# RalphAS/PeriodicSchurDecompositions.jl

Measured on AMD Instinct MI355X. Metric: PSD sweeps/sec (pschur! n=1024 p=64 Float64, Hessenberg+Q+iteration, operands in HBM), higher is better.
Workload: dtype f64

## Files before the change

### periodicschurdecompositions.jl_amd/csrc/psd_engine.cpp

```cpp
#include <atomic>
#include "psd_hess.h"
#include "psd_bhess.h"
#include "psd_hess2.h"
#include "psd_formq2.h"
#include "psd_real_qr.h"
#include "psd_apply2.h"
#include "psd_zhess.h"
#include "psd_zhess2.h"
#include "psd_zqz.h"
#include "psd_zord.h"
#include "psd_rord.h"
#include "psd_rgz.h"
#include "psd_zgz.h"
#include "psd_zgord.h"
#include "psd_grord.h"
#include "psd_rhessx.h"
#include "psd_check.h"
#include "psd_krylov.h"
#include "psd_evec.h"
#include "psd_gevec.h"
#include "psd_bevec.h"

#include "../../include/psd_mi355x.h"

// ... 193 lines not shown
    int hess_graph_n = 0, hess_graph_p = 0;
    double* h2ring = nullptr;
    int h2ring_n = 0;
    double* zh2ring = nullptr;
    int zh2ring_n = 0;
    std::vector<hipEvent_t> h2ev;
    int hess_async = -1;
    int hess_lookahead = 1;
    int hess_xcd = 1;
#endif
    int shard_rank = 0, shard_world = 1;
    int batch_group = 0;
    int bh_nmax = PSD_BH_NMAX;
    int bev_nmax = PSD_BEV_NMAX;
    void slice(int p, int& lo, int& hi) const {
        const int base = p / shard_world, rem = p % shard_world;
        lo = shard_rank * base + (shard_rank < rem ? shard_rank : rem);
        hi = lo + base + (shard_rank < rem ? 1 : 0);
    }
    int train_stop = 1;
    int train_wdiv = 0;
    int train_long = 256;
    int band_helper = 1;
    int zstream = 3;
    int zcdefer = 0;
    int redge = 0, cedge = 0;
    int rdefer = 1;
    int cdefer = 1;
    int overlap = 3;
    int far_grid = 0;
    bool counted = false;
    bool pipe_ok = false;
#ifndef PSD_HOSTSIM
    hipStream_t stream2 = nullptr;
    hipStream_t stream3 = nullptr;
    hipStream_t stream4 = nullptr;
    int hess_pipe_depth = 3;
    int hess_pipe = 1;
    hipEvent_t evE[2] = {nullptr, nullptr}, evF[2] = {nullptr, nullptr}, evG[2] = {nullptr, nullptr};
    hipEvent_t evC[2] = {nullptr, nullptr};
#endif
    int apply_worklist = 1;
    int apply_wl_grid = 2048;
    int ncu = 0;
    int slices = 1;
    unsigned char* slmem = nullptr;
// ... 778 lines not shown
        PSD_CHECK(hipFuncSetAttribute(reinterpret_cast<const void*>(psd_rq_step),
                                      hipFuncAttributeMaxDynamicSharedMemorySize, (int)lds_step));
        c->step_lds_set = lds_step;
    }
#endif
    const int M = (c->train_m >= 2) ? ((c->train_m > PSD_TRAIN_MAX) ? PSD_TRAIN_MAX : c->train_m) : 1;
    P.cst = nullptr;
    P.tshift = nullptr;
    P.lead = c->st;
    P.tick = 0;
    P.gl = nullptr;
    P.cep = nullptr;
    P.role = P.epoch = P.cdone = nullptr;
    P.nprob = 1;
    P.ticklog = nullptr;
    P.ticklog_n = 0;
    P.bandinfo = nullptr;
    P.ccancel = nullptr;
    P.plan = nullptr;
    const bool scan3 = c->chase3 && p >= PSD_C3_MINP && p <= PSD_C3_MAXP;
    P.c2off = (scan3 || (c->chase2 && p >= PSD_C2_MINP)) ? (int)((size_t)p * psd_win_area(W) * sizeof(double)) : 0;
    P.c3off = scan3 ? (int)step_lds_scratch_end(p, W, 8, true) : 0;
    P.cdefer = 0;
    P.slG = 1;
    P.slmem = nullptr;
    P.slerr = nullptr;
    const int c2waves = scan3 ? PSD_C3_WAVES : (P.c2off ? 2 : 1);
    (void)c2waves;
    struct ExitGuard {
        psd_ctx* c;
        int** ticklog;
        ~ExitGuard() {
#ifndef PSD_HOSTSIM
            if (c->stream2) (void)hipStreamSynchronize(c->stream2);
#endif
            if (*ticklog) {
                psd_rt_free(*ticklog);
                *ticklog = nullptr;
            }
        }
    } exit_guard{c, &P.ticklog};
    const char* ticklog_path = psd_env_diag("PSD_TICKLOG");
    const int ticklog_cap = 1 << 16;
    if (ticklog_path && nprob == 1) {
        if (psd_rt_malloc((void**)&P.ticklog, sizeof(int) * ticklog_cap) == 0) {
            PSD_CHECK(psd_rt_memset(P.ticklog, 0, sizeof(int) * ticklog_cap, c->stream));
// ... 299 lines not shown
#endif
#ifndef PSD_HOSTSIM
    PSD_CHECK(poller.finish(pend));
#endif
    PSD_CHECK(psd_rt_last_error());
#ifndef PSD_HOSTSIM
    if (slG > 1) {
        int serr = 0;
        PSD_CHECK(psd_rt_d2h(&serr, P.slerr, sizeof(int), c->stream));
        PSD_CHECK(psd_rt_sync(c->stream));
        if (serr) {
            *st_out = hst;
            return PSD_INFO_RUNTIME + 0xfffa;
        }
    }
#endif
    if (P.ticklog) {
        std::vector<int> tl((size_t)ticklog_cap);
        PSD_CHECK(psd_rt_d2h(tl.data(), P.ticklog, sizeof(int) * ticklog_cap, c->stream));
        PSD_CHECK(psd_rt_sync(c->stream));
        fprintf(stderr, "psd ticklog: phase cycles (decide, spawn, train shifts, small QR, claims, cursor states, deflate, RQ window):");
        for (int q = 0; q < 8; ++q) fprintf(stderr, " %lld/%d", hgl.dbg[q], hgl.dbgn[q]);
        fprintf(stderr, "\n");
        if (hgl.c3dbg[7] > 0) {
            fprintf(stderr, "psd ticklog: scan chase, cycles per position (loads + scan 1, reflectors + B, scan 2, 2-reflectors + records, barrier, apply 0, apply 1) over %lld positions:", hgl.c3dbg[7]);
            for (int q = 0; q < 7; ++q) fprintf(stderr, " %.0f", (double)hgl.c3dbg[q] / (double)hgl.c3dbg[7]);
            fprintf(stderr, "\n");
        }
        if (FILE* fh = fopen(ticklog_path, "w")) {
            for (long long t = 0; t < launched && t < ticklog_cap; ++t) fprintf(fh, "%lld %d %d\n", t, tl[(size_t)t] >> 12, tl[(size_t)t] & 0xfff);
            fclose(fh);
        }
    }
    *st_out = hst;
    if (stats) {
        stats->nlaunch_step = (int32_t)launched;
        stats->window = W;
        stats->step_kernel_ms_avg = samples ? sample_ms / samples : 0.0;
        stats->step_kernel_samples = samples;
    }
    return 0;
}

void stats_from_state(psd_stats* s, const psd_rstate& st) {
    if (!s) return;
    s->niter = st.niter;
// ... 121 lines not shown
        if (const char* e = psd_env("PSD_H2_PIPE")) c->hess_pipe = atoi(e);
        if (const char* e = psd_env("PSD_H2_DEPTH")) c->hess_pipe_depth = atoi(e);
    }
#endif
#ifndef PSD_HOSTSIM
    if (const char* e = psd_env("PSD_HESS_LOOKAHEAD")) c->hess_lookahead = atoi(e);
    if (const char* e = psd_env("PSD_HESS_ASYNC")) c->hess_async = atoi(e);
#endif
#ifdef PSD_HOSTSIM
    if (const char* e = psd_env("PSD_OVERLAP")) c->overlap = atoi(e);
#endif
    if (const char* e = psd_env("PSD_CDEFER")) c->cdefer = atoi(e);
    if (const char* e = psd_env("PSD_RDEFER")) c->rdefer = atoi(e);
    if (const char* e = psd_env("PSD_ZCDEFER")) c->zcdefer = atoi(e);
    if (const char* e = psd_env("PSD_ZSTREAM")) c->zstream = atoi(e);
    if (const char* e = psd_env("PSD_RDEFER_EDGE")) c->redge = atoi(e);
    if (const char* e = psd_env("PSD_CDEFER_EDGE")) c->cedge = atoi(e);
    if (const char* e = psd_env("PSD_ORD_PIPE")) c->ord_pipe = atoi(e);
    if (const char* e = psd_env("PSD_FORMQ_BLOCKED")) c->formq_blocked = atoi(e);
    if (const char* e = psd_env("PSD_BATCH_GROUP")) c->batch_group = atoi(e) > 0 ? atoi(e) : 0;
    if (const char* e = psd_env_diag("PSD_BH_NMAX")) c->bh_nmax = (atoi(e) >= 1 && atoi(e) <= 2048) ? atoi(e) : PSD_BH_NMAX;
    if (const char* e = psd_env_diag("PSD_BEV_NMAX")) c->bev_nmax = (atoi(e) >= 1 && atoi(e) <= 2048) ? atoi(e) : PSD_BEV_NMAX;
    if (const char* e = psd_env("PSD_BAND_HELPER")) c->band_helper = atoi(e);
    if (const char* e = psd_env_diag("PSD_TRAIN_LONG")) c->train_long = atoi(e);
    if (const char* e = psd_env_diag("PSD_TRAIN_STOP")) c->train_stop = atoi(e);
    if (const char* e = psd_env_diag("PSD_TRAIN_WDIV")) c->train_wdiv = atoi(e) > 0 ? atoi(e) : 0;
    if (const char* e = psd_env("PSD_MB")) c->mblock = atoi(e);
    if (const char* e = psd_env_diag("PSD_TRAIN_MB")) c->train_mb_m = atoi(e);
    if (const char* e = psd_env_diag("PSD_APPLY_WL")) c->apply_worklist = atoi(e);
    if (const char* e = psd_env_diag("PSD_APPLY_WL_GRID")) c->apply_wl_grid = atoi(e) > 0 ? atoi(e) : 2048;
    if (const char* e = psd_env_diag("PSD_APPLY_WL2")) c->apply_wl2 = atoi(e);
    if (const char* e = psd_env("PSD_C2")) c->chase2 = atoi(e);
    if (const char* e = psd_env("PSD_C3")) c->chase3 = atoi(e);
#ifndef PSD_HOSTSIM
#endif
    if (const char* e = psd_env_diag("PSD_APPLY_WL2_GRID")) c->apply_wl2_grid = atoi(e) > 0 ? atoi(e) : 1024;
#ifdef PSD_HOSTSIM
    c->apply_wl_grid = 3;
#endif
    if (const char* e = psd_env("PSD_TRAIN")) c->train_m = c->ztrain_m = c->gtrain_m = atoi(e);
    if (const char* e = psd_env("PSD_TRAIN_Z")) c->ztrain_m = atoi(e);
    if (const char* e = psd_env("PSD_TRAIN_G")) c->gtrain_m = atoi(e);
    c->counted = true;
    c->pipe_ok = g_live_contexts.fetch_add(1) == 0;
    *ctx = c;
    return 0;
// ... 2244 lines not shown
```

### periodicschurdecompositions.jl_amd/csrc/psd_real_qr.h

```cpp
#pragma once
#include "psd_scalar.h"
#include "psd_hqr.h"

enum {
    PSD_PH_DECIDE = 0,
    PSD_PH_RQ = 1,
    PSD_PH_SHIFT = 2,
    PSD_PH_QR = 3,
    PSD_PH_DEFLATE = 4,
    PSD_PH_NEXT = 5,
    PSD_PH_FINAL = 6,
    PSD_PH_DONE = 7,
    PSD_PH_TWAIT = 8,
    PSD_PH_CWAIT = 9,
    PSD_PH_CDONE = 10
};
enum { PSD_TR_R3 = 3, PSD_TR_H2 = 2, PSD_TR_R2 = 4, PSD_TR_G = 5 };

#define PSD_TR_CAP 64
#define PSD_STEP_NT 64
#define PSD_APPLY_NT 128
#define PSD_TRAIN_MAX 64
#define PSD_SLOTS 64
enum { PSD_ROLE_FREE = 0, PSD_ROLE_CLAIMED = 1, PSD_ROLE_LEADER = 2, PSD_ROLE_CURSOR = 3 };
// ... 71 lines not shown
    int exc_dec;
    int mb, slot, parent, lo, train_key;
    int prob;
    int cgap, tgap, cstart, cfirst;
    int cslots[PSD_TRAIN_MAX];
    int train_S, train_ms, train_long, train_wdiv;
    int plan_tick, plan_used;
    int opn_tick;
};

struct psd_rglobal {
    int done, info, abort;
    int nactive;
    int nlog;
    int train_seq;
    int itbudget;
    int pactive[PSD_SLOTS], pbudget[PSD_SLOTS], pinfo[PSD_SLOTS];
    int nsweeps, nrqpass, ndefl1, ndefl2, nwindows, ntrains, ntrainsweeps, maxits, nspawn, nslotmax;
    long long niter;
    long long cyc[6];
    long long dbg[8];
    int dbgn[8];
    long long c3dbg[8];
};

struct psd_rparams {
    double* H;
    double* Z;
    psd_rstate* st;
    psd_apply_desc* desc;
    psd_tr* tr;
    int* cnt;
    double* hdiag;
    double* hsub;
    double* hsup;
    double* Pd;
    double* Pe;
    double* Pf;
    double* hnorms;
    double* wr;
    double* wi;
    int* log;
    psd_rstate* cst;
    double* tshift;
    psd_rstate* lead;
    int tick;
    psd_rglobal* gl;
    int* cep;
    int* role;
    int* epoch;
    int nprob;
    int* cdone;
    int* ticklog;
    int ticklog_n;
    int* bandinfo;
    int* ccancel;
    int* plan;
    int c2off;
    int c3off;
    int slG;
    unsigned char* slmem;
    int* slerr;
    int cdefer;
    int redge, cedge;
};
PSD_HD int psd_cdefer_edge(int Wmax) { return (Wmax + 2 > 16) ? (Wmax + 2) : 16; }
PSD_HD int psd_rdefer_edge(int Wmax) { return (2 * Wmax + 8 > 48) ? (2 * Wmax + 8) : 48; }
#define PSD_PLAN_FIRST 0
#define PSD_PLAN_COUNT (PSD_SLOTS)
#define PSD_PLAN_FREE (2 * PSD_SLOTS)
#define PSD_PLAN_CDONE (3 * PSD_SLOTS)
#define PSD_PLAN_CCANCEL (4 * PSD_SLOTS)
#define PSD_PLAN_TICK (5 * PSD_SLOTS)
#define PSD_PLAN_INTS (5 * PSD_SLOTS + 8)
#define PSD_TSHIFT_STRIDE (4 * PSD_TRAIN_MAX + 8)
#define PSD_TRAIN_LONG_MINW 64
#define PSD_DECIDE_YIELD 128

#define PSD_DBG_T0() const long long _dbg0 = (P.ticklog != nullptr) ? psd_clock() : 0
#define PSD_DBG_ADD(k)                                                        \
    do {                                                                      \
        if (P.ticklog != nullptr && P.gl != nullptr) {                        \
            PSD_ONE {                                                         \
                psd_atomic_add_ll(&P.gl->dbg[k], psd_clock() - _dbg0);        \
                psd_atomic_add(&P.gl->dbgn[k], 1);                            \
            }                                                                 \
        }                                                                     \
    } while (0)
PSD_HD psd_mat<double> psd_fac(const psd_rparams& P, int n, int j) {
    return psd_mat<double>{P.H + (size_t)(j - 1) * n * n, n};
}

PSD_HD int psd_win_area(int Wmax) { return Wmax * ((((Wmax + 1) & 1) == 0) ? (Wmax + 1) : (Wmax + 2)); }
PSD_HD int psd_win_pitch(int W, int Wmax) {
    if (((W + 1) & 1) == 0) return W + 1;
    return (W * (W + 2) <= psd_win_area(Wmax)) ? (W + 2) : (W + 1);
}
struct psd_win {
    double* b;
    int W, ld, bsz, bs, be;
    PSD_HD double& at(int j, int r, int c) const { return b[(j - 1) * bsz + (c - bs) * ld + (r - bs)]; }
};

#define PSD_WIN_BAND 3
#define PSD_WIN_LF 4
struct alignas(8) psd_pair {
    double a, b;
};
#ifdef PSD_HOSTSIM
PSD_D psd_pair psd_pair_load(const double* q) { return *(const psd_pair*)q; }
PSD_D void psd_pair_store(double* q, const psd_pair& x) { *(psd_pair*)q = x; }
// ... 430 lines not shown
        const int a = a0 + t;
        if (a <= i) {
            double d = 1.0, e = 0.0, f = 0.0;
            for (int j = 2; j <= p; ++j) {
                const psd_mat<double> Hj = psd_mat<double>{H + (size_t)(j - 1) * n * n, n};
                if (a + 2 <= i) f = d * Hj(a, a + 2) + e * Hj(a + 1, a + 2) + f * Hj(a + 2, a + 2);
                if (a + 1 <= i) e = d * Hj(a, a + 1) + e * Hj(a + 1, a + 1);
                d *= Hj(a, a);
            }
            P.Pd[sb + a] = d;
            P.Pe[sb + a] = e;
            P.Pf[sb + a] = f;
        }
    }
    if (chunk == 0) {
        PSD_ONE {
            P.bandinfo[s] = P.tick;
            P.bandinfo[PSD_SLOTS + s] = lo;
            P.bandinfo[2 * PSD_SLOTS + s] = i;
        }
    }
}

PSD_D double psd_h1_opnorm(const psd_rparams& P, const psd_rstate& st, double* red, int lo, int hi) {
    const psd_mat<double> H1 = psd_fac(P, st.n, 1);
    const int NT = PSD_NTHREADS;
    PSD_PAR_FOR(t, NT) {
        double best = 0.0;
        for (int c = lo + t; c <= hi; c += NT) {
            double s = 0.0;
            const int rmax = (c + 1 < hi) ? (c + 1) : hi;
            for (int r = lo; r <= rmax; ++r) s += fabs(H1(r, c));
            if (s > best) best = s;
        }
        red[t] = best;
    }
    PSD_SYNC();
    double best = 0.0;
    for (int t = 0; t < NT; ++t)
        if (red[t] > best) best = red[t];
    PSD_SYNC();
    return best;
}

PSD_D bool psd_rq_decide(const psd_rparams& P, psd_rstate& st, double* red, int* redi, double* stage, size_t stage_doubles) {
    const int n = st.n, p = st.p, i = st.i, lo = st.l;
    const int NT = PSD_NTHREADS;
    if (!(st.its < st.maxitleft)) {
        if (st.mb && P.nprob > 1) {
            PSD_ONE { psd_atomic_store(&P.gl->pinfo[st.prob], i); }
            st.phase = PSD_PH_FINAL;
            return false;
        }
        st.info = i;
        st.phase = PSD_PH_DONE;
        if (st.mb) {
            PSD_ONE {
                psd_atomic_store(&P.gl->info, i);
                psd_atomic_store(&P.gl->pinfo[st.prob], i);
                psd_atomic_store(&P.gl->abort, 1);
                psd_atomic_store(&P.gl->done, 1);
            }
        }
        return false;
    }
    const psd_mat<double> H1 = psd_fac(P, n, 1);
    bool have = false;
    if (P.bandinfo != nullptr && st.mb) {
        have = P.bandinfo[st.slot] == P.tick && P.bandinfo[PSD_SLOTS + st.slot] <= lo && i <= P.bandinfo[2 * PSD_SLOTS + st.slot];
    }
    if (!have) {
        const int pj = p - 1;
        int R = (pj > 0) ? (int)(stage_doubles / (3 * (size_t)pj)) - 2 : NT;
        if (R > NT) R = NT;
        if (pj > 0 && R >= 1) {
            for (int a0 = lo; a0 <= i; a0 += R) {
                const int a1 = (a0 + R - 1 < i) ? (a0 + R - 1) : i;
                const int c1 = (a1 + 2 < i) ? (a1 + 2) : i;
                const int nc = c1 - a0 + 1;
                PSD_SYNC();
                PSD_PAR_FOR(t, nc * pj) {
                    const int cc = t % nc, jj = t / nc;
                    const int c = a0 + cc;
                    const psd_mat<double> Hj = psd_fac(P, n, jj + 2);
                    double* q = stage + 3 * (size_t)t;
                    q[0] = Hj(c, c);
                    q[1] = (c - 1 >= lo) ? Hj(c - 1, c) : 0.0;
                    q[2] = (c - 2 >= lo) ? Hj(c - 2, c) : 0.0;
                }
// ... 9 lines not shown
                    }
                    P.Pd[a] = d;
                    P.Pe[a] = e;
                    P.Pf[a] = f;
                }
            }
        } else {
            PSD_PAR_FOR(t, i - lo + 1) {
                const int a = lo + t;
                double d = 1.0, e = 0.0, f = 0.0;
                for (int j = 2; j <= p; ++j) {
                    const psd_mat<double> Hj = psd_fac(P, n, j);
                    if (a + 2 <= i) f = d * Hj(a, a + 2) + e * Hj(a + 1, a + 2) + f * Hj(a + 2, a + 2);
                    if (a + 1 <= i) e = d * Hj(a, a + 1) + e * Hj(a + 1, a + 1);
                    d *= Hj(a, a);
                }
                P.Pd[a] = d;
                P.Pe[a] = e;
                P.Pf[a] = f;
            }
        }
    }
    PSD_SYNC();
    PSD_PAR_FOR(t, i - lo + 1) {
        const int r = lo + t;
        if (i == lo) {
            P.hdiag[i] = H1(i, i) * P.Pd[i];
        } else if (r == i) {
            P.hsub[i] = H1(i, i - 1) * P.Pd[i - 1];
            P.hdiag[i] = H1(i, i - 1) * P.Pe[i - 1] + H1(i, i) * P.Pd[i];
        } else if (r > lo) {
            P.hsub[r] = H1(r, r - 1) * P.Pd[r - 1];
            P.hdiag[r] = H1(r, r - 1) * P.Pe[r - 1] + H1(r, r) * P.Pd[r];
            P.hsup[r] = H1(r, r - 1) * P.Pf[r - 1] + H1(r, r) * P.Pe[r] + H1(r, r + 1) * P.Pd[r + 1];
        } else {
            P.hdiag[r] = H1(r, r) * P.Pd[r];
            P.hsup[r] = H1(r, r) * P.Pe[r] + H1(r, r + 1) * P.Pd[r + 1];
        }
    }
    PSD_SYNC();
    int klast = 0;
    double h1norm = -1.0;
    for (int pass = 0; pass < 2; ++pass) {
        PSD_PAR_FOR(t, NT) {
            int best = 0, need = 0;
            for (int k = i - t; k >= lo + 1; k -= NT) {
                const double hh21 = P.hsub[k], hh22 = P.hdiag[k], hh11 = P.hdiag[k - 1], hh12 = P.hsup[k - 1];
                double tst1 = fabs(hh11) + fabs(hh22);
                if (tst1 == 0) {
                    if (h1norm < 0) {
                        need = 1;
                        continue;
                    }
                    tst1 = h1norm;
                }
                bool found = false;
                if (fabs(hh21) <= st.smlnum) {
                    found = true;
                } else if (fabs(hh21) <= st.ulp * tst1) {
                    const double ab = fmax(fabs(hh21), fabs(hh12));
                    const double ba = fmin(fabs(hh21), fabs(hh12));
                    const double aa = fmax(fabs(hh22), fabs(hh11 - hh22));
                    const double bb = fmin(fabs(hh22), fabs(hh11 - hh22));
                    const double stmp = aa + ab;
                    found = ba * (ab / stmp) <= fmax(st.smlnum, st.ulpx * (bb * (aa / stmp)));
                }
                if (found) {
                    best = k;
                    break;
                }
            }
            redi[t] = best;
            redi[NT + t] = need;
        }
        PSD_SYNC();
        int need = 0;
        klast = 0;
        for (int t = 0; t < NT; ++t) {
            if (redi[t] > klast) klast = redi[t];
            need |= redi[NT + t];
        }
        PSD_SYNC();
        if (!need) break;
        if (P.cdefer && st.opn_tick != P.tick - 1) {
            st.opn_tick = P.tick;
            return true;
        }
        h1norm = psd_h1_opnorm(P, st, red, lo, i);
    }
    const bool found = klast > 0;
    const int l = (i > lo) ? (found ? klast : lo) : i;
    st.l = l;
    st.phase = PSD_PH_SHIFT;
    if (l > 1 && st.wantT) {
        double tst1 = fabs(H1(l - 1, l - 1)) + fabs(H1(l, l));
        if (tst1 == 0) {
            if (P.cdefer && st.opn_tick != P.tick - 1) {
                st.opn_tick = P.tick;
                st.l = lo;
                st.phase = PSD_PH_DECIDE;
                return true;
            }
            tst1 = psd_h1_opnorm(P, st, red, l, i);
        }
        if (fabs(H1(l, l - 1)) > fmax(st.ulp * tst1, st.smlnum)) {
            st.phase = PSD_PH_RQ;
            st.kcur = i;
            st.nrqpass += 1;
            psd_log(P, st, 1, l, i);
        } else {
            PSD_SYNC();
            PSD_ONE { H1(l, l - 1) = 0.0; }
            PSD_SYNC();
        }
    }
    return false;
}


PSD_D void psd_rq_startvec(const double h11, const double h12, const double h21, const double h22, const double h32,
                           const double* sh, double* v) {
    const double rt1r = sh[0], rt1i = sh[1], rt2r = sh[2], rt2i = sh[3];
    const double s = fabs(h11 - rt2r) + fabs(rt2i) + fabs(h21);
    const double h21s = h21 / s;
    const double v1 = h21s * h12 + (h11 - rt1r) * ((h11 - rt2r) / s) - rt1i * (rt2i / s);
    const double v2 = h21s * (h11 + h22 - rt1r - rt2r);
    const double v3 = h21s * h32;
    const double t = fabs(v1) + fabs(v2) + fabs(v3);
    v[0] = v1 / t;
    v[1] = v2 / t;
    v[2] = v3 / t;
}

PSD_D void psd_rq_topband(const psd_rparams& P, int n, int p, int l, int i, double& h11, double& h12, double& h21,
                          double& h22, double& h32) {
    double d0 = 1.0, e0 = 0.0, d1 = 1.0;
    for (int j = 2; j <= p; ++j) {
// ... 4 lines not shown
    }
    const psd_mat<double> H1 = psd_fac(P, n, 1);
    h11 = H1(l, l) * d0;
    h12 = H1(l, l) * e0 + H1(l, l + 1) * d1;
    h21 = H1(l + 1, l) * d0;
    h22 = H1(l + 1, l) * e0 + H1(l + 1, l + 1) * d1;
    h32 = (l + 2 <= i) ? H1(l + 2, l + 1) * d1 : 0.0;
}

PSD_HD size_t psd_rq_train_doubles(int p, int m) {
    const size_t K = 2 * (size_t)m, K1 = K + 1;
    return (size_t)p * K1 * K1 + 2 * K1 * K1 + K * K + 3 * PSD_HQR_MAX + 8;
}
PSD_D void psd_rq_train_shifts(const psd_rparams& P, int n, int p, int i, int m, double* work, int* okf) {
    const int K = 2 * m, K1 = K + 1, t0 = i - K + 1, KK = K1 * K1;
    double* B = work;
    double* R0 = B + (size_t)p * KK;
    double* R1 = R0 + KK;
    double* T = R1 + KK;
    double* wr = T + K * K;
    double* wi = wr + PSD_HQR_MAX;
    double* re = wi + PSD_HQR_MAX;
    PSD_SYNC();
    PSD_PAR_FOR(t, p * KK) {
        const int j = t / KK, q = t - j * KK, r = q / K1, c = q - r * K1;
        B[t] = psd_fac(P, n, j + 1)(t0 - 1 + r, t0 - 1 + c);
    }
    PSD_PAR_FOR(q, KK) { R0[q] = (q / K1 == q % K1) ? 1.0 : 0.0; }
    PSD_SYNC();
    double* cur = R0;
    double* nxt = R1;
    for (int j = 2; j <= p; ++j) {
        const double* Bj = B + (size_t)(j - 1) * KK;
        PSD_PAR_FOR(q, KK) {
            const int r = q / K1, c = q - r * K1;
            double acc = 0.0;
            for (int k = r; k <= c; ++k) acc += cur[r * K1 + k] * Bj[k * K1 + c];
            nxt[q] = acc;
        }
        PSD_SYNC();
        double* sw = cur;
        cur = nxt;
        nxt = sw;
    }
    PSD_PAR_FOR(q, K * K) {
        const int r = q / K, c = q - r * K;
        double acc = 0.0;
        for (int k = r; k <= c + 1; ++k) acc += B[(r + 1) * K1 + k] * cur[k * K1 + (c + 1)];
        T[q] = acc;
    }
    PSD_SYNC();
#ifndef PSD_HOSTSIM
    const long long _hq0 = psd_clock();
    const bool okw = psd_hqr_wave(T, K, K, wr, wi, PSD_TID);
    if (P.ticklog != nullptr && P.gl != nullptr) {
        PSD_ONE {
            psd_atomic_add_ll(&P.gl->dbg[3], psd_clock() - _hq0);
            psd_atomic_add(&P.gl->dbgn[3], 1);
        }
    }
#endif
    PSD_ONE {
#ifndef PSD_HOSTSIM
        bool ok = okw;
#else
        bool ok = psd_hqr(T, K, K, wr, wi);
#endif
        int np = 0, nre = 0;
        for (int q = 0; ok && q < K; ++q) {
            if (!(wr[q] == wr[q]) || !(wi[q] == wi[q])) ok = false;
            if (wi[q] > 0.0) {
                if (np < m) {
// ... 14 lines not shown
            }
            re[b + 1] = x;
        }
        for (int a = 0; ok && a < nre && np < m; a += 2) {
            double* sh = P.tshift + 4 * np;
            sh[0] = re[a]; sh[1] = 0.0; sh[2] = (a + 1 < nre) ? re[a + 1] : re[a]; sh[3] = 0.0;
            ++np;
        }
        *okf = (ok && np == m) ? 1 : 0;
    }
    PSD_SYNC();
}

PSD_HD void psd_cursor_schedule(const psd_rstate& st, int b, int& cstart, int& cfirst) {
    const int nbw = st.W - 4;
    const int spc = (st.tgap == 1) ? (nbw + 4) : (2 * nbw);
    int d = (b * spc - nbw + 1 + nbw - 1) / nbw;
    if (d < 1) d = 1;
    int x = nbw * d - b * spc + nbw;
    if (x > nbw) x = nbw;
    if (x < 1) x = 1;
    cstart = st.train_tick0 + d;
    cfirst = x;
}

PSD_D bool psd_rq_shift(const psd_rparams& P, psd_rstate& st, double* work, int* bc) {
    const int n = st.n, i = st.i, l = st.l;
    bool heavy = false;
    if (st.mb && st.l > st.lo && st.l < i - 1) {
        PSD_DBG_T0();
        psd_mb_spawn(P, st, bc);
        PSD_DBG_ADD(1);
    }
    if (l >= i - 1) {
        st.phase = PSD_PH_DEFLATE;
        return false;
    }
    if (!st.wantT) {
        st.i1 = l;
        st.i2 = i;
    }
    psd_log(P, st, 0, l, i);
    st.nsweeps += 1;
    const double dat1 = 0.75, dat2 = -0.4375;
    const double* hdiag = P.hdiag;
    const double* hsub = P.hsub;
// ... 172 lines not shown
            const double h44s = h44 - h11, h33s = h33 - h11;
            v1 = (h33s * h44s - h43h34) / h21 + h12;
            v2 = h22 - h11 - h33s - h44s;
            v3 = hsub[m + 2];
        } else {
            const double s = fabs(h11 - rt2r) + fabs(rt2i) + fabs(h21);
            const double h21s = h21 / s;
            v1 = h21s * h12 + (h11 - rt1r) * ((h11 - rt2r) / s) - rt1i * (rt2i / s);
            v2 = h21s * (h11 + h22 - rt1r - rt2r);
            v3 = h21s * hsub[m + 2];
        }
        const double s = fabs(v1) + fabs(v2) + fabs(v3);
        st.v[0] = v1 / s;
        st.v[1] = v2 / s;
        st.v[2] = v3 / s;
    }
    st.phase = PSD_PH_QR;
    st.kcur = l;
    if (st.train_n > 1) {
        PSD_DBG_T0();
        PSD_SYNC();
        PSD_ONE {
            if (!st.mb) psd_atomic_store(P.cep + PSD_TRAIN_MAX, 0);
            const int ngen1 = (st.mb && st.train_S > 0 && st.train_S + 1 < st.train_n) ? (st.train_S + 1) : st.train_n;
            for (int b = 1; b < ngen1; ++b) {
                psd_rstate cs = st;
                cs.cursor = b;
                cs.phase = PSD_PH_CWAIT;
                cs.kcur = 0;
                cs.nsweeps = cs.nwindows = cs.nlog = 0;
                cs.maxlog = 0;
                for (int q = 0; q < 6; ++q) cs.cyc[q] = 0;
                psd_cursor_schedule(st, b, cs.cstart, cs.cfirst);
                if (st.mb) {
                    cs.parent = st.slot;
                    cs.slot = st.cslots[b];
                    P.cst[cs.slot] = cs;
                    psd_atomic_store(P.epoch + cs.slot, P.tick);
                } else {
                    psd_pub_begin(P.cep + b);
                    P.cst[b] = cs;
                    psd_pub_end(P.cep + b, P.tick);
                }
            }
        }
        PSD_SYNC();
        PSD_DBG_ADD(5);
    }
    return heavy;
}

PSD_D void psd_desc_write(const psd_rparams& P, psd_rstate& st, const int* lcnt, int plo, int phi, int lc0,
                          int lc1, int rr0, int rr1, int split = 0) {
    PSD_SYNC();
    const bool over = psd_list_overflow(lcnt, st.p, PSD_TR_CAP);
    if (over) {
        st.info = PSD_LIST_OVERFLOW;
        st.phase = PSD_PH_DONE;
        if (st.mb) {
            PSD_ONE {
                psd_atomic_store(&P.gl->info, PSD_LIST_OVERFLOW);
                psd_atomic_store(&P.gl->abort, 1);
                psd_atomic_store(&P.gl->done, 1);
            }
        }
    }
// ... 520 lines not shown
    PSD_LDS_DECL;
    psd_c2* cmd = (psd_c2*)(psd_lds + P.c2off);
    C.cmd = 1;
    PSD_ONE { *cmd = C; }
    PSD_PAIR_BARRIER();
    psd_c2_run(C, 1);
    PSD_ONE { cmd->cmd = 0; }
#endif
}
#ifndef PSD_HOSTSIM
PSD_D void psd_c3_run(const psd_c2& Cin, int wv_, int nw_, int taboff_);
PSD_D void psd_c3s_run(const psd_c2& Cin, int wv_, int nw_, int taboff_);
PSD_D void psd_c2_helper(int c2off, int c3off) {
    PSD_LDS_DECL;
    const psd_c2* cmd = (const psd_c2*)(psd_lds + c2off);
    for (;;) {
        PSD_PAIR_BARRIER();
        const psd_c2 C = *cmd;
        if (C.cmd == 0) return;
        if (C.cmd == 2) {
            psd_c3_run(C, PSD_WAVE_ROLE, (int)blockDim.y, c3off);
        } else if (C.cmd == 5) {
            psd_c3s_run(C, PSD_WAVE_ROLE, (int)blockDim.y, c3off);
        } else if (C.cmd == 3 || C.cmd == 4) {
            psd_rparams R;
            R.H = C.H;
            psd_win w;
            w.b = (double*)(psd_lds + C.wboff);
            w.W = C.W; w.ld = C.ld; w.bsz = C.bsz; w.bs = C.bs; w.be = C.be;
            if (C.cmd == 3) psd_win_load(R, w, C.n, C.p, PSD_WAVE_ROLE, (int)blockDim.y);
            else psd_win_store(R, w, C.n, C.p, PSD_WAVE_ROLE, (int)blockDim.y);
            PSD_PAIR_BARRIER();
        } else {
            psd_c2_run(C, 2);
        }
    }
}
PSD_D void psd_c2_release(int c2off) {
    PSD_LDS_DECL;
    psd_c2* cmd = (psd_c2*)(psd_lds + c2off);
    PSD_ONE { cmd->cmd = 0; }
    PSD_PAIR_BARRIER();
}
#endif

#include "psd_chase3.h"
// ... 572 lines not shown
    PSD_LDS_DECL;
    psd_rstate st = *P.st;
    if (st.phase == PSD_PH_DONE) {
        PSD_ONE { P.desc->active = 0; }
        return;
    }
    const int NT = PSD_NTHREADS;
    double* ldsd = (double*)psd_lds;
    const size_t winb = (size_t)st.p * psd_win_area(st.Wmax);
    double* red = ldsd + winb;
    int* redi = (int*)(red + NT);
    int* lcnt = redi + 2 * NT;
    PSD_ONE { P.desc->active = 0; }
    const long long tk0 = psd_clock(), tw0 = psd_wallclock();
    bool emitted = false;
    int guard = 0;
    int phmask = 0;
    while (!emitted && st.phase != PSD_PH_DONE && guard < 4 * st.n + 16) {
        ++guard;
        phmask |= 1 << st.phase;
        switch (st.phase) {
            case PSD_PH_DECIDE: {
                const long long td0 = psd_clock();
                {
                    PSD_DBG_T0();
                    if (psd_rq_decide(P, st, red, redi, ldsd, winb)) emitted = true;
                    PSD_DBG_ADD(0);
                }
                st.cyc[0] += psd_clock() - td0;

                break;
            }
            case PSD_PH_RQ: {
                PSD_DBG_T0();
                psd_rq_rq_window(P, st, ldsd, lcnt);
                PSD_DBG_ADD(7);
                emitted = true;
                break;
            }
            case PSD_PH_SHIFT:
                if (psd_rq_shift(P, st, ldsd, redi)) emitted = true;
                break;
            case PSD_PH_QR:
                psd_rq_qr_window(P, st, ldsd, lcnt);
                emitted = true;
                break;
// ... 846 lines not shown
```

Before: 2466.

## Spread deflation decision work across helper waves of the workgroup

Adds a job-dispatch path (command 6) so the helper waves already parked in the chase-helper loop also take part in the RQ decision work. With it they build the band tridiagonal, run the negligible-subdiagonal search, and form the trailing periodic product for the shifts. Cursor-state generation for the train also moves from a single thread to a parallel loop. The goal is to cut serial latency in the decide and shift phases by using idle waves, at the cost of extra barriers, LDS job blocks and new per-phase diagnostic counters.

```diff
diff --git a/periodicschurdecompositions.jl_amd/csrc/psd_engine.cpp b/periodicschurdecompositions.jl_amd/csrc/psd_engine.cpp
--- a/periodicschurdecompositions.jl_amd/csrc/psd_engine.cpp
+++ b/periodicschurdecompositions.jl_amd/csrc/psd_engine.cpp
@@ -239,6 +239,7 @@
     int train_wdiv = 0;
     int train_long = 256;
     int band_helper = 1;
+    int decide_wg = 1;
     int zstream = 3;
     int zcdefer = 0;
     int redge = 0, cedge = 0;
@@ -1063,6 +1064,7 @@
     P.c2off = (scan3 || (c->chase2 && p >= PSD_C2_MINP)) ? (int)((size_t)p * psd_win_area(W) * sizeof(double)) : 0;
     P.c3off = scan3 ? (int)step_lds_scratch_end(p, W, 8, true) : 0;
     P.cdefer = 0;
+    P.dwg = c->decide_wg;
     P.slG = 1;
     P.slmem = nullptr;
     P.slerr = nullptr;
@@ -1408,6 +1410,9 @@
         fprintf(stderr, "psd ticklog: phase cycles (decide, spawn, train shifts, small QR, claims, cursor states, deflate, RQ window):");
         for (int q = 0; q < 8; ++q) fprintf(stderr, " %lld/%d", hgl.dbg[q], hgl.dbgn[q]);
         fprintf(stderr, "\n");
+        fprintf(stderr, "psd ticklog: decision cycles (band + tridiagonal, deflation search, opnorm, RQ decision, trailing blocks staged, trailing product):");
+        for (int q = 0; q < 6; ++q) fprintf(stderr, " %lld/%d", hgl.dbg2[q], hgl.dbgn2[q]);
+        fprintf(stderr, " | launches %lld, with a deciding leader %d\n", launched, hgl.declaunch);
         if (hgl.c3dbg[7] > 0) {
             fprintf(stderr, "psd ticklog: scan chase, cycles per position (loads + scan 1, reflectors + B, scan 2, 2-reflectors + records, barrier, apply 0, apply 1) over %lld positions:", hgl.c3dbg[7]);
             for (int q = 0; q < 7; ++q) fprintf(stderr, " %.0f", (double)hgl.c3dbg[q] / (double)hgl.c3dbg[7]);
@@ -1575,6 +1580,7 @@
     if (const char* e = psd_env_diag("PSD_BH_NMAX")) c->bh_nmax = (atoi(e) >= 1 && atoi(e) <= 2048) ? atoi(e) : PSD_BH_NMAX;
     if (const char* e = psd_env_diag("PSD_BEV_NMAX")) c->bev_nmax = (atoi(e) >= 1 && atoi(e) <= 2048) ? atoi(e) : PSD_BEV_NMAX;
     if (const char* e = psd_env("PSD_BAND_HELPER")) c->band_helper = atoi(e);
+    if (const char* e = psd_env("PSD_DECIDE_WG")) c->decide_wg = atoi(e) ? 1 : 0;
     if (const char* e = psd_env_diag("PSD_TRAIN_LONG")) c->train_long = atoi(e);
     if (const char* e = psd_env_diag("PSD_TRAIN_STOP")) c->train_stop = atoi(e);
     if (const char* e = psd_env_diag("PSD_TRAIN_WDIV")) c->train_wdiv = atoi(e) > 0 ? atoi(e) : 0;
diff --git a/periodicschurdecompositions.jl_amd/csrc/psd_real_qr.h b/periodicschurdecompositions.jl_amd/csrc/psd_real_qr.h
--- a/periodicschurdecompositions.jl_amd/csrc/psd_real_qr.h
+++ b/periodicschurdecompositions.jl_amd/csrc/psd_real_qr.h
@@ -117,6 +117,9 @@
     long long dbg[8];
     int dbgn[8];
     long long c3dbg[8];
+    long long dbg2[8];
+    int dbgn2[8];
+    int declaunch, dectick;
 };
 
 struct psd_rparams {
@@ -158,6 +161,7 @@
     int* slerr;
     int cdefer;
     int redge, cedge;
+    int dwg;
 };
 PSD_HD int psd_cdefer_edge(int Wmax) { return (Wmax + 2 > 16) ? (Wmax + 2) : 16; }
 PSD_HD int psd_rdefer_edge(int Wmax) { return (2 * Wmax + 8 > 48) ? (2 * Wmax + 8) : 48; }
@@ -182,6 +186,23 @@
             }                                                                 \
         }                                                                     \
     } while (0)
+#ifdef PSD_DIAG
+#define PSD_DBG2_ON(P) ((P).ticklog != nullptr && (P).gl != nullptr)
+#define PSD_DBG2_T0() const long long _dbg2 = PSD_DBG2_ON(P) ? psd_clock() : 0
+#define PSD_DBG2_ADD(k)                                                       \
+    do {                                                                      \
+        if (PSD_DBG2_ON(P)) {                                                 \
+            PSD_ONE {                                                         \
+                psd_atomic_add_ll(&P.gl->dbg2[k], psd_clock() - _dbg2);       \
+                psd_atomic_add(&P.gl->dbgn2[k], 1);                           \
+            }                                                                 \
+        }                                                                     \
+    } while (0)
+#else
+#define PSD_DBG2_ON(P) false
+#define PSD_DBG2_T0() ((void)0)
+#define PSD_DBG2_ADD(k) ((void)0)
+#endif
 PSD_HD psd_mat<double> psd_fac(const psd_rparams& P, int n, int j) {
     return psd_mat<double>{P.H + (size_t)(j - 1) * n * n, n};
 }
@@ -658,6 +679,199 @@
     }
 }
 
+enum { PSD_DW_BAND = 1, PSD_DW_SEARCH = 2, PSD_DW_SHIFTS = 3 };
+struct psd_dw {
+    int job;
+    int n, p, lo, i;
+    int soff;
+    int K, dbgon;
+    double h1norm, smlnum, ulp, ulpx;
+    double* H;
+    double *Pd, *Pe, *Pf, *hdiag, *hsub, *hsup;
+    long long* dbg2;
+};
+#define PSD_DW_SIMWAVES 4
+#define PSD_DW_OFF 256
+#ifdef PSD_HOSTSIM
+#define PSD_WG_FOR(t, count, wv, nw)                                                      \
+    for (int t##_0 = (wv) * 64; t##_0 < (int)(count); t##_0 += (nw) * 64)                 \
+        for (int t = t##_0; t < t##_0 + 64 && t < (int)(count); ++t)
+#define PSD_DW_BARRIER() ((void)0)
+#define PSD_DW_NW PSD_DW_SIMWAVES
+#else
+#define PSD_DW_NW ((int)blockDim.y)
+#define PSD_WG_FOR(t, count, wv, nw) for (int t = (wv) * 64 + (int)threadIdx.x; t < (int)(count); t += (nw) * 64)
+#define PSD_DW_BARRIER()                                               \
+    do {                                                               \
+        __builtin_amdgcn_fence(__ATOMIC_RELEASE, "workgroup");         \
+        asm volatile("s_waitcnt vmcnt(0) lgkmcnt(0)" ::: "memory");    \
+        __builtin_amdgcn_s_barrier();                                  \
+        __builtin_amdgcn_fence(__ATOMIC_ACQUIRE, "workgroup");         \
+    } while (0)
+#endif
+PSD_D bool psd_dw_on(const psd_rparams& P) {
+#ifdef PSD_HOSTSIM
+    return P.dwg != 0 && P.c3off != 0;
+#else
+    return P.dwg != 0 && P.c3off != 0 && blockDim.y > 1;
+#endif
+}
+
+PSD_D void psd_rq_tri_row(const psd_mat<double>& H1, const double* Pd, const double* Pe, const double* Pf, double* hdiag,
+                          double* hsub, double* hsup, int lo, int i, int r) {
+    if (i == lo) {
+        hdiag[i] = H1(i, i) * Pd[i];
+    } else if (r == i) {
+        hsub[i] = H1(i, i - 1) * Pd[i - 1];
+        hdiag[i] = H1(i, i - 1) * Pe[i - 1] + H1(i, i) * Pd[i];
+    } else if (r > lo) {
+        hsub[r] = H1(r, r - 1) * Pd[r - 1];
+        hdiag[r] = H1(r, r - 1) * Pe[r - 1] + H1(r, r) * Pd[r];
+        hsup[r] = H1(r, r - 1) * Pf[r - 1] + H1(r, r) * Pe[r] + H1(r, r + 1) * Pd[r + 1];
+    } else {
+        hdiag[r] = H1(r, r) * Pd[r];
+        hsup[r] = H1(r, r) * Pe[r] + H1(r, r + 1) * Pd[r + 1];
+    }
+}
+PSD_D int psd_rq_negl(const double* hsub, const double* hdiag, const double* hsup, int k, double smlnum, double ulp,
+                      double ulpx, double h1norm) {
+    const double hh21 = hsub[k], hh22 = hdiag[k], hh11 = hdiag[k - 1], hh12 = hsup[k - 1];
+    double tst1 = fabs(hh11) + fabs(hh22);
+    if (tst1 == 0) {
+        if (h1norm < 0) return 2;
+        tst1 = h1norm;
+    }
+    bool found = false;
+    if (fabs(hh21) <= smlnum) {
+        found = true;
+    } else if (fabs(hh21) <= ulp * tst1) {
+        const double ab = fmax(fabs(hh21), fabs(hh12));
+        const double ba = fmin(fabs(hh21), fabs(hh12));
+        const double aa = fmax(fabs(hh22), fabs(hh11 - hh22));
+        const double bb = fmin(fabs(hh22), fabs(hh11 - hh22));
+        const double stmp = aa + ab;
+        found = ba * (ab / stmp) <= fmax(smlnum, ulpx * (bb * (aa / stmp)));
+    }
+    return found ? 1 : 0;
+}
+PSD_D double psd_ts_prod(const double* cur, const double* Bj, int K1, int q) {
+    const int r = q / K1, c = q - r * K1;
+    double acc = 0.0;
+    for (int k = r; k <= c; ++k) acc += cur[r * K1 + k] * Bj[k * K1 + c];
+    return acc;
+}
+PSD_D double psd_ts_top(const double* B, const double* cur, int K, int K1, int q) {
+    const int r = q / K, c = q - r * K;
+    double acc = 0.0;
+    for (int k = r; k <= c + 1; ++k) acc += B[(r + 1) * K1 + k] * cur[k * K1 + (c + 1)];
+    return acc;
+}
+
+PSD_HD int psd_dw_phases(const psd_dw& D) { return (D.job == PSD_DW_SHIFTS) ? (D.p + 1) : 1; }
+PSD_D void psd_dw_phase(const psd_dw& D, int ph, int wv, int nw) {
+    PSD_LDS_DECL;
+    const int lo = D.lo, i = D.i;
+    if (D.job == PSD_DW_BAND) {
+        const psd_mat<double> H1 = psd_mat<double>{D.H, D.n};
+        PSD_WG_FOR(t, i - lo + 1, wv, nw) { psd_rq_tri_row(H1, D.Pd, D.Pe, D.Pf, D.hdiag, D.hsub, D.hsup, lo, i, lo + t); }
+    } else if (D.job == PSD_DW_SEARCH) {
+        int* ri = (int*)(psd_lds + D.soff);
+        PSD_WG_FOR(t, 64 * nw, wv, nw) {
+            const int c = t & 63, sq = t >> 6;
+            int best = 0, zmax = 0;
+            for (int k = i - c - 64 * sq; k >= lo + 1; k -= 64 * nw) {
+                const int v = psd_rq_negl(D.hsub, D.hdiag, D.hsup, k, D.smlnum, D.ulp, D.ulpx, D.h1norm);
+                if (v == 2 && zmax == 0) zmax = k;
+                if (v == 1) {
+                    best = k;
+                    break;
+                }
+            }
+            ri[t] = best;
+            ri[64 * nw + t] = zmax;
+        }
+    } else if (D.job == PSD_DW_SHIFTS) {
+        const int p = D.p, K = D.K, K1 = K + 1, t0 = i - K + 1, KK = K1 * K1;
+        double* B = (double*)(psd_lds + D.soff);
+        double* R0 = B + (size_t)p * KK;
+        double* R1 = R0 + KK;
+        double* T = R1 + KK;
+        if (ph == 0) {
+            PSD_WG_FOR(t, p * KK, wv, nw) {
+                const int j = t / KK, q = t - j * KK, r = q / K1, c = q - r * K1;
+                B[t] = psd_mat<double>{D.H + (size_t)j * D.n * D.n, D.n}(t0 - 1 + r, t0 - 1 + c);
+            }
+            PSD_WG_FOR(q, KK, wv, nw) { R0[q] = (q / K1 == q % K1) ? 1.0 : 0.0; }
+        } else if (ph < p) {
+            const double* cur = (ph & 1) ? R0 : R1;
+            double* nxt = (ph & 1) ? R1 : R0;
+            const double* Bj = B + (size_t)ph * KK;
+            PSD_WG_FOR(q, KK, wv, nw) { nxt[q] = psd_ts_prod(cur, Bj, K1, q); }
+        } else {
+            const double* cur = ((p - 1) & 1) ? R1 : R0;
+            PSD_WG_FOR(q, K * K, wv, nw) { T[q] = psd_ts_top(B, cur, K, K1, q); }
+        }
+    }
+}
+PSD_D void psd_dw_exec(const psd_dw& D, int wv, int nw) {
+#ifdef PSD_HOSTSIM
+    (void)wv;
+    for (int ph = 0; ph < psd_dw_phases(D); ++ph)
+        for (int g = 0; g < nw; ++g) psd_dw_phase(D, ph, g, nw);
+#else
+    const int nph = psd_dw_phases(D);
+    long long tq = (D.dbgon && wv == 0) ? psd_clock() : 0;
+    for (int ph = 0; ph < nph; ++ph) {
+        psd_dw_phase(D, ph, wv, nw);
+        PSD_DW_BARRIER();
+        if (D.dbgon && wv == 0 && D.job == PSD_DW_SHIFTS && (ph == 0 || ph == nph - 1)) {
+            const long long tn = psd_clock();
+            if (threadIdx.x == 0) psd_atomic_add_ll(D.dbg2 + ((ph == 0) ? 4 : 5), tn - tq);
+            tq = tn;
+        }
+    }
+#endif
+}
+PSD_D void psd_dw_run(const psd_rparams& P, psd_dw& D) {
+    D.dbgon = 0;
+    D.dbg2 = nullptr;
+#ifdef PSD_DIAG
+    if (PSD_DBG2_ON(P)) {
+        D.dbgon = 1;
+        D.dbg2 = P.gl->dbg2;
+    }
+#endif
+#ifdef PSD_HOSTSIM
+    psd_dw_exec(D, 0, PSD_DW_SIMWAVES);
+#else
+    PSD_LDS_DECL;
+    int* cmdw = (int*)(psd_lds + P.c2off);
+    psd_dw* job = (psd_dw*)(psd_lds + P.c2off + PSD_DW_OFF);
+    PSD_SYNC();
+    PSD_ONE {
+        *job = D;
+        *cmdw = 6;
+    }
+    PSD_PAIR_BARRIER();
+    psd_dw_exec(D, 0, (int)blockDim.y);
+    PSD_ONE { *cmdw = 0; }
+#endif
+}
+PSD_D void psd_dw_search_reduce(const int* ri, int nw, int& klast, int& need) {
+    klast = 0;
+    need = 0;
+    for (int c = 0; c < 64; ++c) {
+        int best = 0, zmax = 0;
+        for (int sq = 0; sq < nw; ++sq) {
+            const int b = ri[64 * sq + c], z = ri[64 * nw + 64 * sq + c];
+            if (b > best) best = b;
+            if (z > zmax) zmax = z;
+        }
+        if (best > klast) klast = best;
+        if (zmax > best) need = 1;
+    }
+}
+
 PSD_D double psd_h1_opnorm(const psd_rparams& P, const psd_rstate& st, double* red, int lo, int hi) {
     const psd_mat<double> H1 = psd_fac(P, st.n, 1);
     const int NT = PSD_NTHREADS;
@@ -701,6 +915,7 @@
         return false;
     }
     const psd_mat<double> H1 = psd_fac(P, n, 1);
+    PSD_DBG2_T0();
     bool have = false;
     if (P.bandinfo != nullptr && st.mb) {
         have = P.bandinfo[st.slot] == P.tick && P.bandinfo[PSD_SLOTS + st.slot] <= lo && i <= P.bandinfo[2 * PSD_SLOTS + st.slot];
@@ -756,77 +971,79 @@
         }
     }
     PSD_SYNC();
-    PSD_PAR_FOR(t, i - lo + 1) {
-        const int r = lo + t;
-        if (i == lo) {
-            P.hdiag[i] = H1(i, i) * P.Pd[i];
-        } else if (r == i) {
-            P.hsub[i] = H1(i, i - 1) * P.Pd[i - 1];
-            P.hdiag[i] = H1(i, i - 1) * P.Pe[i - 1] + H1(i, i) * P.Pd[i];
-        } else if (r > lo) {
-            P.hsub[r] = H1(r, r - 1) * P.Pd[r - 1];
-            P.hdiag[r] = H1(r, r - 1) * P.Pe[r - 1] + H1(r, r) * P.Pd[r];
-            P.hsup[r] = H1(r, r - 1) * P.Pf[r - 1] + H1(r, r) * P.Pe[r] + H1(r, r + 1) * P.Pd[r + 1];
-        } else {
-            P.hdiag[r] = H1(r, r) * P.Pd[r];
-            P.hsup[r] = H1(r, r) * P.Pe[r] + H1(r, r + 1) * P.Pd[r + 1];
-        }
+    const bool wide = psd_dw_on(P) && i - lo + 1 > NT;
+    psd_dw D;
+    if (wide) {
+        PSD_LDS_DECL;
+        D.n = n; D.p = p; D.lo = lo; D.i = i;
+        D.soff = (int)((char*)stage - (char*)psd_lds);
+        D.K = 0;
+        D.h1norm = -1.0; D.smlnum = st.smlnum; D.ulp = st.ulp; D.ulpx = st.ulpx;
+        D.H = P.H;
+        D.Pd = P.Pd; D.Pe = P.Pe; D.Pf = P.Pf; D.hdiag = P.hdiag; D.hsub = P.hsub; D.hsup = P.hsup;
+    }
+    if (wide) {
+        D.job = PSD_DW_BAND;
+        psd_dw_run(P, D);
+    } else {
+        PSD_PAR_FOR(t, i - lo + 1) { psd_rq_tri_row(H1, P.Pd, P.Pe, P.Pf, P.hdiag, P.hsub, P.hsup, lo, i, lo + t); }
     }
     PSD_SYNC();
+    PSD_DBG2_ADD(0);
     int klast = 0;
     double h1norm = -1.0;
     for (int pass = 0; pass < 2; ++pass) {
-        PSD_PAR_FOR(t, NT) {
-            int best = 0, need = 0;
-            for (int k = i - t; k >= lo + 1; k -= NT) {
-                const double hh21 = P.hsub[k], hh22 = P.hdiag[k], hh11 = P.hdiag[k - 1], hh12 = P.hsup[k - 1];
-                double tst1 = fabs(hh11) + fabs(hh22);
-                if (tst1 == 0) {
-                    if (h1norm < 0) {
-                        need = 1;
-                        continue;
+        int need = 0;
+        {
+            PSD_DBG2_T0();
+            if (wide) {
+                D.job = PSD_DW_SEARCH;
+                D.h1norm = h1norm;
+                psd_dw_run(P, D);
+                psd_dw_search_reduce((const int*)stage, PSD_DW_NW, klast, need);
+                PSD_SYNC();
+            } else {
+                PSD_PAR_FOR(t, NT) {
+                    int best = 0, nd = 0;
+                    for (int k = i - t; k >= lo + 1; k -= NT) {
+                        const int v = psd_rq_negl(P.hsub, P.hdiag, P.hsup, k, st.smlnum, st.ulp, st.ulpx, h1norm);
+                        if (v == 2) {
+                            nd = 1;
+                            continue;
+                        }
+                        if (v == 1) {
+                            best = k;
+                            break;
+                        }
                     }
-                    tst1 = h1norm;
-                }
-                bool found = false;
-                if (fabs(hh21) <= st.smlnum) {
-                    found = true;
-                } else if (fabs(hh21) <= st.ulp * tst1) {
-                    const double ab = fmax(fabs(hh21), fabs(hh12));
-                    const double ba = fmin(fabs(hh21), fabs(hh12));
-                    const double aa = fmax(fabs(hh22), fabs(hh11 - hh22));
-                    const double bb = fmin(fabs(hh22), fabs(hh11 - hh22));
-                    const double stmp = aa + ab;
-                    found = ba * (ab / stmp) <= fmax(st.smlnum, st.ulpx * (bb * (aa / stmp)));
-                }
-                if (found) {
-                    best = k;
-                    break;
-                }
-            }
-            redi[t] = best;
-            redi[NT + t] = need;
-        }
-        PSD_SYNC();
-        int need = 0;
-        klast = 0;
-        for (int t = 0; t < NT; ++t) {
-            if (redi[t] > klast) klast = redi[t];
-            need |= redi[NT + t];
-        }
-        PSD_SYNC();
+                    redi[t] = best;
+                    redi[NT + t] = nd;
+                }
+                PSD_SYNC();
+                klast = 0;
+                for (int t = 0; t < NT; ++t) {
+                    if (redi[t] > klast) klast = redi[t];
+                    need |= redi[NT + t];
+                }
+                PSD_SYNC();
+            }
+            PSD_DBG2_ADD(1);
+        }
         if (!need) break;
         if (P.cdefer && st.opn_tick != P.tick - 1) {
             st.opn_tick = P.tick;
             return true;
         }
+        PSD_DBG2_T0();
         h1norm = psd_h1_opnorm(P, st, red, lo, i);
+        PSD_DBG2_ADD(2);
     }
     const bool found = klast > 0;
     const int l = (i > lo) ? (found ? klast : lo) : i;
     st.l = l;
     st.phase = PSD_PH_SHIFT;
     if (l > 1 && st.wantT) {
+        PSD_DBG2_T0();
         double tst1 = fabs(H1(l - 1, l - 1)) + fabs(H1(l, l));
         if (tst1 == 0) {
             if (P.cdefer && st.opn_tick != P.tick - 1) {
@@ -847,6 +1064,7 @@
             PSD_ONE { H1(l, l - 1) = 0.0; }
             PSD_SYNC();
         }
+        PSD_DBG2_ADD(3);
     }
     return false;
 }
@@ -897,32 +1115,49 @@
     double* wi = wr + PSD_HQR_MAX;
     double* re = wi + PSD_HQR_MAX;
     PSD_SYNC();
-    PSD_PAR_FOR(t, p * KK) {
-        const int j = t / KK, q = t - j * KK, r = q / K1, c = q - r * K1;
-        B[t] = psd_fac(P, n, j + 1)(t0 - 1 + r, t0 - 1 + c);
-    }
-    PSD_PAR_FOR(q, KK) { R0[q] = (q / K1 == q % K1) ? 1.0 : 0.0; }
-    PSD_SYNC();
-    double* cur = R0;
-    double* nxt = R1;
-    for (int j = 2; j <= p; ++j) {
-        const double* Bj = B + (size_t)(j - 1) * KK;
-        PSD_PAR_FOR(q, KK) {
-            const int r = q / K1, c = q - r * K1;
-            double acc = 0.0;
-            for (int k = r; k <= c; ++k) acc += cur[r * K1 + k] * Bj[k * K1 + c];
-            nxt[q] = acc;
-        }
-        PSD_SYNC();
-        double* sw = cur;
-        cur = nxt;
-        nxt = sw;
-    }
-    PSD_PAR_FOR(q, K * K) {
-        const int r = q / K, c = q - r * K;
-        double acc = 0.0;
-        for (int k = r; k <= c + 1; ++k) acc += B[(r + 1) * K1 + k] * cur[k * K1 + (c + 1)];
-        T[q] = acc;
+    if (psd_dw_on(P)) {
+        PSD_LDS_DECL;
+        psd_dw D;
+        D.job = PSD_DW_SHIFTS;
+        D.n = n; D.p = p; D.lo = 0; D.i = i;
+        D.soff = (int)((char*)work - (char*)psd_lds);
+        D.K = K;
+        D.h1norm = 0.0; D.smlnum = 0.0; D.ulp = 0.0; D.ulpx = 0.0;
+        D.H = P.H;
+        D.Pd = D.Pe = D.Pf = D.hdiag = D.hsub = D.hsup = nullptr;
+        psd_dw_run(P, D);
+#ifdef PSD_DIAG
+        if (PSD_DBG2_ON(P)) {
+            PSD_ONE {
+                psd_atomic_add(&P.gl->dbgn2[4], 1);
+                psd_atomic_add(&P.gl->dbgn2[5], 1);
+            }
+        }
+#endif
+    } else {
+        {
+            PSD_DBG2_T0();
+            PSD_PAR_FOR(t, p * KK) {
+                const int j = t / KK, q = t - j * KK, r = q / K1, c = q - r * K1;
+                B[t] = psd_fac(P, n, j + 1)(t0 - 1 + r, t0 - 1 + c);
+            }
+            PSD_PAR_FOR(q, KK) { R0[q] = (q / K1 == q % K1) ? 1.0 : 0.0; }
+            PSD_SYNC();
+            PSD_DBG2_ADD(4);
+        }
+        PSD_DBG2_T0();
+        double* cur = R0;
+        double* nxt = R1;
+        for (int j = 2; j <= p; ++j) {
+            const double* Bj = B + (size_t)(j - 1) * KK;
+            PSD_PAR_FOR(q, KK) { nxt[q] = psd_ts_prod(cur, Bj, K1, q); }
+            PSD_SYNC();
+            double* sw = cur;
+            cur = nxt;
+            nxt = sw;
+        }
+        PSD_PAR_FOR(q, K * K) { T[q] = psd_ts_top(B, cur, K, K1, q); }
+        PSD_DBG2_ADD(5);
     }
     PSD_SYNC();
 #ifndef PSD_HOSTSIM
@@ -983,6 +1218,27 @@
     if (x < 1) x = 1;
     cstart = st.train_tick0 + d;
     cfirst = x;
+}
+
+PSD_D void psd_rq_cursor_state(const psd_rparams& P, const psd_rstate& st, int b) {
+    psd_rstate cs = st;
+    cs.cursor = b;
+    cs.phase = PSD_PH_CWAIT;
+    cs.kcur = 0;
+    cs.nsweeps = cs.nwindows = cs.nlog = 0;
+    cs.maxlog = 0;
+    for (int q = 0; q < 6; ++q) cs.cyc[q] = 0;
+    psd_cursor_schedule(st, b, cs.cstart, cs.cfirst);
+    if (st.mb) {
+        cs.parent = st.slot;
+        cs.slot = st.cslots[b];
+        P.cst[cs.slot] = cs;
+        psd_atomic_store(P.epoch + cs.slot, P.tick);
+    } else {
+        psd_pub_begin(P.cep + b);
+        P.cst[b] = cs;
+        psd_pub_end(P.cep + b, P.tick);
+    }
 }
 
 PSD_D bool psd_rq_shift(const psd_rparams& P, psd_rstate& st, double* work, int* bc) {
@@ -1201,26 +1457,13 @@
         PSD_SYNC();
         PSD_ONE {
             if (!st.mb) psd_atomic_store(P.cep + PSD_TRAIN_MAX, 0);
-            const int ngen1 = (st.mb && st.train_S > 0 && st.train_S + 1 < st.train_n) ? (st.train_S + 1) : st.train_n;
-            for (int b = 1; b < ngen1; ++b) {
-                psd_rstate cs = st;
-                cs.cursor = b;
-                cs.phase = PSD_PH_CWAIT;
-                cs.kcur = 0;
-                cs.nsweeps = cs.nwindows = cs.nlog = 0;
-                cs.maxlog = 0;
-                for (int q = 0; q < 6; ++q) cs.cyc[q] = 0;
-                psd_cursor_schedule(st, b, cs.cstart, cs.cfirst);
-                if (st.mb) {
-                    cs.parent = st.slot;
-                    cs.slot = st.cslots[b];
-                    P.cst[cs.slot] = cs;
-                    psd_atomic_store(P.epoch + cs.slot, P.tick);
-                } else {
-                    psd_pub_begin(P.cep + b);
-                    P.cst[b] = cs;
-                    psd_pub_end(P.cep + b, P.tick);
-                }
+        }
+        const int ngen1 = (st.mb && st.train_S > 0 && st.train_S + 1 < st.train_n) ? (st.train_S + 1) : st.train_n;
+        if (P.dwg) {
+            PSD_PAR_FOR(b1, ngen1 - 1) { psd_rq_cursor_state(P, st, b1 + 1); }
+        } else {
+            PSD_ONE {
+                for (int b = 1; b < ngen1; ++b) psd_rq_cursor_state(P, st, b);
             }
         }
         PSD_SYNC();
@@ -1787,6 +2030,11 @@
             psd_c3_run(C, PSD_WAVE_ROLE, (int)blockDim.y, c3off);
         } else if (C.cmd == 5) {
             psd_c3s_run(C, PSD_WAVE_ROLE, (int)blockDim.y, c3off);
+        } else if (C.cmd == 6) {
+            static_assert(sizeof(psd_c2) <= PSD_DW_OFF && PSD_DW_OFF + sizeof(psd_dw) <= PSD_STEP_NT * sizeof(double),
+                          "command and job block share the reduction scratch");
+            const psd_dw D = *(const psd_dw*)(psd_lds + c2off + PSD_DW_OFF);
+            psd_dw_exec(D, PSD_WAVE_ROLE, (int)blockDim.y);
         } else if (C.cmd == 3 || C.cmd == 4) {
             psd_rparams R;
             R.H = C.H;
@@ -2405,6 +2653,13 @@
         switch (st.phase) {
             case PSD_PH_DECIDE: {
                 const long long td0 = psd_clock();
+#ifdef PSD_DIAG
+                if (PSD_DBG2_ON(P)) {
+                    PSD_ONE {
+                        if (psd_atomic_max(&P.gl->dectick, P.tick + 1) < P.tick + 1) psd_atomic_add(&P.gl->declaunch, 1);
+                    }
+                }
+#endif
                 {
                     PSD_DBG_T0();
                     if (psd_rq_decide(P, st, red, redi, ldsd, winb)) emitted = true;
```

After: 2483, median of 2. No clear change (+0.7%).
